# hall-lab/svtyper

Measured on AMD Instinct MI355X. Metric: breakpoints genotyped/sec, higher is better.
Workload: dtype f64

## Files before the change

### svtyper_amd/csrc/svt_batch_create.h

```cpp

struct StageTimer {
    bool on = std::getenv("SVT_TRACE") != nullptr;
    std::chrono::steady_clock::time_point t0 = std::chrono::steady_clock::now();
    void mark(const char* what)
    {
        if (!on) return;
        const auto t1 = std::chrono::steady_clock::now();
        std::fprintf(stderr, "[svt] %-28s %8.2f ms\n", what, std::chrono::duration<double, std::milli>(t1 - t0).count());
        t0 = t1;
    }
};

int record_error(uint32_t err_bits)
{
    return fail(SVT_ERR_INVALID, record_error_text(err_bits));
}

int check_stream_errors(svt_batch* b)
{
    if (b->layout != kLayoutStream || !b->d_err) return SVT_OK;
    uint32_t bits = 0;
    HIP_TRY(hipMemcpyAsync(&bits, b->d_err, sizeof(uint32_t), hipMemcpyDeviceToHost, b->stream));
    HIP_TRY(hipStreamSynchronize(b->stream));
    return bits ? record_error(bits) : SVT_OK;
// ... 310 lines not shown
    tables = (tables + 127) & ~size_t(127);
    if (single) {
        int wgs = 3;
        hipFuncAttributes fa{};
        if (hipFuncGetAttributes(&fa, stream_kernel_of(b, 1)) == hipSuccess && fa.numRegs > 0) wgs = std::max(1, std::min(8, 512 / ((fa.numRegs + 7) / 8 * 8)));
        else (void)hipGetLastError();
        const size_t by_lds = (160 * 1024) / (tables + kWavesPerBlock * kStreamRingBytes);
        b->one_tile_round_units = (uint64_t)std::min<size_t>((size_t)wgs, std::max<size_t>(by_lds, 1)) * cu_count(b->device) * kBlock;
    }
    {
        int wgs = 3;
        hipFuncAttributes fa{};
        if (hipFuncGetAttributes(&fa, b->mode == kMultiLds ? window_budget_kernel() : stream_kernel_of(b, tiles_per_wave(b, n))) == hipSuccess && fa.numRegs > 0)
            wgs = std::max(1, std::min(8, 512 / ((fa.numRegs + 7) / 8 * 8)));
        else
            (void)hipGetLastError();
        if (const char* e = std::getenv("SVT_STREAM_WGS_PER_CU")) wgs = std::max(1, std::atoi(e));
#ifdef SVT_FORCE_WGS
        wgs = SVT_FORCE_WGS;
#endif
        kStreamLdsPerWg = (160 * 1024 / (size_t)wgs) & ~size_t(127);
        b->wgs_per_cu = wgs;
    }
    const size_t l10_bytes = ((size_t)n_l10 * 8 + 127) & ~size_t(127);
    const size_t base_lds = tables + kWavesPerBlock * kStreamRingBytes;
    const size_t fit = std::max<size_t>(1, std::min<size_t>((size_t)b->wgs_per_cu, (160 * 1024) / base_lds));
    const size_t budget = ((160 * 1024) / fit) & ~size_t(127);
    (void)kStreamLdsPerWg;
    if (base_lds + l10_bytes <= budget) {
        a.l10_where = kL10Shared;
        a.lds_l10 = (uint32_t)tables;
        a.l10_lds_entries = n_l10;
        tables += l10_bytes;
    } else if (kStreamDepth == 1 && SVT_L10_THROUGH_RING) {
        a.l10_where = kL10Ring;
        a.l10_lds_entries = (uint32_t)std::min<uint64_t>((n_l10 + 127u) / 128u * 128u, kStreamRingBytes / 8);
    } else {
        a.l10_where = kL10Global;
        a.l10_lds_entries = 0;
    }
    a.lds_rings = (uint32_t)tables;
    if (b->mode == kSingleLds && a.l10_where != kL10Ring) {
        const size_t tab = (a.lds_winlibs + 127) & ~size_t(127);
        b->coop = small_region(tab, kCoopRegionBytes, true, l10_bytes, n_l10);
        if (b->coop.lds_bytes) {
            int wgs = 2;
            hipFuncAttributes fa{};
            if (hipFuncGetAttributes(&fa, coop_kernel_of(b)) == hipSuccess && fa.numRegs > 0) wgs = std::max(1, std::min(4, 512 / ((fa.numRegs + 7) / 8 * 8) * 4 / kCoopWaves));
            else (void)hipGetLastError();
            b->coop_resident = (uint32_t)std::min<size_t>((size_t)wgs, (160 * 1024) / b->coop.lds_bytes) * cu_count(b->device);
            if (b->coop.lds_bytes > 64 * 1024) HIP_TRY(hipFuncSetAttribute(coop_kernel_of(b), hipFuncAttributeMaxDynamicSharedMemorySize, (int)b->coop.lds_bytes));
        }
        b->split = small_region(tab, kSplitRegionBytes, true, l10_bytes, n_l10);
        if (b->split.lds_bytes > 64 * 1024)
            for (int lanes = 2; lanes <= 4; lanes += 2)
                HIP_TRY(hipFuncSetAttribute(split_kernel_of(b, lanes), hipFuncAttributeMaxDynamicSharedMemorySize, (int)b->split.lds_bytes));
    }
    if (b->mode == kMultiLds && a.l10_where != kL10Ring) {
        b->split = small_region((tables + 127) & ~size_t(127), kSplitRegionBytes, false);
        if (b->split.lds_bytes) {
            b->split.l10_where = a.l10_where;
            b->split.lds_l10 = a.lds_l10;
            b->split.l10_entries = a.l10_lds_entries;
        }
        if (b->split.lds_bytes > 64 * 1024)
            for (int lanes = 2; lanes <= 4; lanes += 2)
                if (lanes == 4 || !(b->flags & SVT_FLAG_SSO_ASSOCIATION))
                    HIP_TRY(hipFuncSetAttribute(split_kernel_of(b, lanes), hipFuncAttributeMaxDynamicSharedMemorySize, (int)b->split.lds_bytes));
    }
    a.n_units = n;
    a.unit_begin = 0;
    a.unit_end = (uint32_t)n;
    a.units_per_wg = (uint32_t)kBlock * (uint32_t)tiles_per_wave(b, n);
    a.result96 = (b->flags & SVT_FLAG_RESULT96) ? 1u : 0u;
    a.slot_begin = 0;
    b->resident_wgs = (uint32_t)std::min<size_t>((size_t)b->wgs_per_cu, (160 * 1024) / (tables + kWavesPerBlock * kStreamRingBytes)) *
                      cu_count(b->device);
    b->out_dev = b->d_out;
    b->out_slots = !a.result96 ? n : b->mode == kMultiLds ? (uint64_t)b->n_chunks * kBlock * (uint64_t)b->window_tiles : slots_of_launch(b, n);
    SVT_TRY(ensure_result_slots(b, b->out_slots));
    a.out = b->d_out;
    a.err = b->d_err;
    a.lib0 = T.libs[0];
    fill_gt_consts(a.c, in->split_weight, in->disc_weight);
    b->out_dev = b->d_out;
    b->lds_bytes = tables + kWavesPerBlock * kStreamRingBytes;
    if (b->lds_bytes > 160 * 1024) return fail(SVT_ERR_INVALID, "LDS budget exceeded");
    if (tm.on)
        std::fprintf(stderr, "[svt] kernel budget: %d workgroups/CU by registers, LDS %zu B/workgroup (%zu fit), log10 table (%u entries) %s (%u entries)\n",
                     b->wgs_per_cu, b->lds_bytes, (size_t)(160 * 1024) / std::max<size_t>(b->lds_bytes, 1), n_l10,
                     a.l10_where == kL10Shared ? "in LDS" : a.l10_where == kL10Ring ? "through the ring" : "through L2", a.l10_lds_entries);
    if (b->lds_bytes > 64 * 1024)
        for (int tiles = 1; tiles <= 2; ++tiles)
            if (b->mode != kGeneral || tiles == 1)
                HIP_TRY(hipFuncSetAttribute(stream_kernel_of(b, tiles), hipFuncAttributeMaxDynamicSharedMemorySize, (int)b->lds_bytes));
    if (b->lds_bytes > 64 * 1024 && b->split_window_kinds)
        for (int kind = 1; kind <= 2; ++kind)
            HIP_TRY(hipFuncSetAttribute(window_kernel_of_kind(kind), hipFuncAttributeMaxDynamicSharedMemorySize, (int)b->lds_bytes));
    return SVT_OK;
}
```

### svtyper_amd/csrc/svt_device_types.h

```cpp
#ifndef SVT_DEVICE_TYPES_H
#define SVT_DEVICE_TYPES_H

#include "svt_common.h"

namespace svt {

struct LibDesc {
    uint32_t tab_off;
    int32_t key_min;
    uint32_t n_bins;
    uint32_t pad;
    double v_nondel;
    double sd2;
};

constexpr uint32_t kHalfwordsPerRow = 8u;

constexpr uint32_t kErrStraddleNoPair = 2u, kErrLibIndex = 4u, kErrReservedBits = 8u, kErrNegativeSpan = 16u;

enum Layout : int {
    kLayoutStream = 3,
    kLayoutPacked = 4
};
struct Bin {
    int32_t thr;
    uint32_t hist;
};

constexpr uint32_t kLdsPm = 0;
constexpr uint32_t kLdsWtab = kLdsPm + 256 * 8;
constexpr uint32_t kLdsWcol = kLdsWtab + 32 * 16;
constexpr uint32_t kLdsWcolC = kLdsWcol + 2 * 32 * 8;
constexpr uint32_t kWcolRef = 32 * 8;
constexpr uint32_t kLdsBins = kLdsWcolC + 2 * 32 * 8;

struct GtConsts {
    double lgp[2][3];
    double lg1p[2][3];
    double ln10;
    double x_uflow;
    double split_weight;
    double disc_weight;
};

struct PairWeights { double w_alt, w_ref; };

enum LibMode : int {
    kSingleLds = 0,
    kMultiLds = 1,
    kGeneral = 2
};

struct WgDesc {
    uint32_t lib_lo, lib_cnt, bin_lo, bin_cnt;
};


}

#endif
```

### svtyper_amd/csrc/svt_host_tables.h

```cpp
#ifndef SVT_HOST_TABLES_H
#define SVT_HOST_TABLES_H

#include "svt_device_types.h"

namespace svt {


inline bool p_concordant_expr(uint32_t h1, uint32_t h2, uint64_t n_total)
{
    const double disc_prior = 0.05;
    const double conc_prior = 1 - disc_prior;
    const double d1 = h1 ? (double)h1 / (double)n_total : 0.0;
    const double d2 = h2 ? (double)h2 / (double)n_total : 0.0;
    const double den = conc_prior * d1 + disc_prior * d2;
    if (den == 0.0) return false;
    const double p = d1 * conc_prior / den;
    return p > 0.5;
}

inline double py_log10(double x) { return std::log(x) / std::log(10.0); }

inline double find_pow10_underflow()
{
    double lo = -330.0, hi = -300.0;
    for (int it = 0; it < 200; ++it) {
        double mid = lo + (hi - lo) / 2;
        if (mid == lo || mid == hi) break;
        if (std::pow(10.0, mid) > 0.0) hi = mid; else lo = mid;
    }
    while (std::pow(10.0, std::nextafter(hi, -INFINITY)) > 0.0) hi = std::nextafter(hi, -INFINITY);
    return hi;
}

inline void fill_gt_consts(GtConsts& c, double split_weight, double disc_weight)
{
    const double p_alt[2][3] = {{1e-3, 0.5, 0.9}, {1e-2, 0.2, 1 / 3.0}};
    for (int d = 0; d < 2; ++d)
        for (int g = 0; g < 3; ++g) {
            c.lgp[d][g] = py_log10(p_alt[d][g]);
            c.lg1p[d][g] = py_log10(1 - p_alt[d][g]);
        }
    c.ln10 = std::log(10.0);
    c.x_uflow = find_pow10_underflow();
    c.split_weight = split_weight;
    c.disc_weight = disc_weight;
}


struct HostTables {
    std::vector<LibDesc> libs;
    std::vector<Bin> bins;
    std::vector<PairWeights> wtab;
    std::vector<double> pm;
    std::vector<double> l10;
    bool fast_geometry = true;
    bool narrow_bins = true;
};

inline int build_tables(const svt_evidence_batch* in, uint64_t max_records_per_unit, HostTables& T)
{
    T.libs.resize(in->n_libs);
    for (uint32_t l = 0; l < in->n_libs; ++l) {
        const svt_library& L = in->libs[l];
        if (!L.hist || L.n_bins == 0) return fail(SVT_ERR_INVALID, "library without histogram");
        if (L.n_bins > (1u << 24)) return fail(SVT_ERR_INVALID, "histogram too wide");
        if (!std::isfinite(L.mean) || !std::isfinite(L.sd)) return fail(SVT_ERR_INVALID, "library moments not finite");
        uint64_t total = 0;
        uint32_t hmax = 0;
        for (uint32_t i = 0; i < L.n_bins; ++i) {
            if (L.hist[i] > 0x7FFFFFFFu) return fail(SVT_ERR_INVALID, "histogram count too large");
            total += L.hist[i];
            hmax = std::max(hmax, L.hist[i]);
        }
        LibDesc d{};
        d.tab_off = (uint32_t)T.bins.size();
        d.key_min = L.key_min;
        d.n_bins = L.n_bins;
        d.v_nondel = L.mean + L.sd * 3;
        d.sd2 = 2 * L.sd;
        T.libs[l] = d;
        if (L.key_min < -(1 << 29) || L.key_min > (1 << 29)) T.fast_geometry = false;
        if (!(std::fabs(d.v_nondel - std::nearbyint(d.v_nondel)) > 4e-6) || !(std::fabs(d.v_nondel) < 1e12))
            T.fast_geometry = false;
        for (uint32_t i = 0; i < L.n_bins; ++i) {
            const uint32_t h1 = L.hist[i];
            int32_t t = -1;
            if (h1 > 0 && total > 0 && p_concordant_expr(h1, 0, total)) {
                uint32_t lo = 0, hi = hmax;
                if (p_concordant_expr(h1, hi, total)) lo = hi;
                else
                    while (hi - lo > 1) {
                        const uint32_t mid = lo + (hi - lo) / 2;
                        if (p_concordant_expr(h1, mid, total)) lo = mid; else hi = mid;
                    }
                t = (int32_t)lo;
            }
            T.bins.push_back(Bin{t, h1});
        }
        T.bins.push_back(Bin{-1, 0u});
        {
            Bin* lb = T.bins.data() + d.tab_off;
            std::vector<uint32_t> vals;
            vals.reserve(2 * (size_t)L.n_bins + 2);
            for (uint32_t i = 0; i <= L.n_bins; ++i) {
                vals.push_back(lb[i].hist);
                if (lb[i].thr >= 0) vals.push_back((uint32_t)lb[i].thr);
            }
            std::sort(vals.begin(), vals.end());
            vals.erase(std::unique(vals.begin(), vals.end()), vals.end());
            auto rank = [&](const uint32_t x) { return (uint32_t)(std::lower_bound(vals.begin(), vals.end(), x) - vals.begin()); };
            for (uint32_t i = 0; i <= L.n_bins; ++i) {
                lb[i].hist = rank(lb[i].hist);
                if (lb[i].thr >= 0) lb[i].thr = (int32_t)rank((uint32_t)lb[i].thr);
            }
            if (vals.size() > 32767) T.narrow_bins = false;
        }
    }
    T.wtab.resize(32);
    for (int i = 0; i < 32; ++i) {
        const bool alt = i & 1, ra = i & 2, rb = i & 4, pc = i & 8, del = i & 16;
        const bool both = ra && rb, any = ra || rb;
        const bool need = any && (!both || del);
        T.wtab[i].w_alt = (alt && !(del && pc)) ? 1.0 : 0.0;
        T.wtab[i].w_ref = (need && pc) ? (both ? 1.0 : 0.5) : 0.0;
    }
    const double bound = 2.0 * (2.0 * in->split_weight + in->disc_weight) * (double)max_records_per_unit + 4.0;
    if (bound > 64.0 * 1024 * 1024) return fail(SVT_ERR_INVALID, "weights * records too large for the log table");
    T.l10.resize((size_t)bound + 1);
    T.l10[0] = 0.0;
    for (size_t i = 1; i < T.l10.size(); ++i) T.l10[i] = py_log10((double)i);
    T.pm.resize(256);
    for (int q = 0; q < 256; ++q) T.pm[q] = 1.0 - std::pow(10.0, -(double)q / 10.0);
    return SVT_OK;
}


}

#endif
```

### svtyper_amd/csrc/svt_stream_kernel.h

```cpp
#ifndef SVT_STREAM_KERNEL_H
#define SVT_STREAM_KERNEL_H

#ifndef SVT_STREAM_AUX
#define SVT_STREAM_AUX 2
#endif
#ifndef SVT_STREAM_EDGE_AUX
#define SVT_STREAM_EDGE_AUX 0
#endif
#ifndef SVT_STREAM_SPLIT
#define SVT_STREAM_SPLIT 4
#endif
#ifndef SVT_STREAM_WAVES
#define SVT_STREAM_WAVES 3
#endif
#ifndef SVT_WINDOW_WAVES
#define SVT_WINDOW_WAVES 3
#endif

#include <type_traits>

#include "svt_wg_parts.h"

namespace svt {

template <int MODE>
struct RecordCheck {
    uint32_t flags_or = 0, span_or = 0, lone = 0, lib_max = 0;
    __device__ __forceinline__ void see(const u32x4 w, const uint32_t lib_key = 0u)
    {
        if (MODE == kMultiLds) flags_or |= w.w ^ lib_key;
        else flags_or |= w.w;
        span_or |= w.x;
        lone = max(lone, (w.w & 0x17u) ^ 0x10u);
        if (MODE == kGeneral) lib_max = max(lib_max, w.w & 0xffff00u);
    }
    __device__ __forceinline__ void window_lib(const uint32_t d) { lib_max = max(lib_max, d); }
    __device__ __forceinline__ uint32_t bits(const uint32_t limit) const
    {
        const uint32_t n_libs = limit;
        const bool bad_lib = MODE == kSingleLds ? (flags_or & 0xffff00u) != 0u
                             : MODE == kMultiLds ? (limit == 1u ? (flags_or & 0xffff00u) != 0u : lib_max >= limit)
                                                 : (lib_max >> SVT_REC_LIB_SHIFT) >= n_libs;
        return (lone > 0x10u ? kErrStraddleNoPair : 0u) | (bad_lib ? kErrLibIndex : 0u) |
               ((flags_or & ~SVT_REC_FLAG_MASK) ? kErrReservedBits : 0u) | ((int32_t)span_or < 0 ? kErrNegativeSpan : 0u);
    }
};

template <bool SSO, bool EDGE, bool CONT = true>
__device__ __forceinline__ double record_weights(const u32x4 w, const bool mine, Acc& a)
{
    const uint32_t wy = EDGE ? (mine ? w.y : 0u) : w.y;
    const uint32_t wz = EDGE ? (mine ? w.z : 0u) : w.z;
    const double pm_a = lds_f64(kSPm + byte0_x8(wy)), pm_b = lds_f64(kSPm + byte1_x8(wy));
    const double rs_a = lds_f64(kSPm + byte2_x8(wy)), rs_b = lds_f64(kSPm + byte3_x8(wy));
    const double p_seq = lds_f64(kSPmHalf + byte0_x8(wz)) + lds_f64(kSPmHalf + byte1_x8(wz));
    const double p_clip = lds_f64(kSPmHalf + byte2_x8(wz)) + lds_f64(kSPmHalf + byte3_x8(wz));
    if (SSO && !CONT) {
        a.ref_seq += a.l_ref_seq;
        a.alt_seq += a.l_alt_seq;
        a.alt_clip += a.l_alt_clip;
        a.l_ref_seq = rs_a + rs_b;
        a.l_alt_seq = p_seq;
        a.l_alt_clip = p_clip;
    } else if (SSO) {
        const bool cont = (w.w & SVT_REC_CONTINUATION) != 0u;
        a.ref_seq += cont ? 0.0 : a.l_ref_seq;
        a.alt_seq += cont ? 0.0 : a.l_alt_seq;
        a.alt_clip += cont ? 0.0 : a.l_alt_clip;
        a.l_ref_seq = ((cont ? a.l_ref_seq : 0.0) + rs_a) + rs_b;
        a.l_alt_seq = (cont ? a.l_alt_seq : 0.0) + p_seq;
        a.l_alt_clip = (cont ? a.l_alt_clip : 0.0) + p_clip;
    } else {
        a.ref_seq = (a.ref_seq + rs_a) + rs_b;
        a.alt_seq += p_seq;
        a.alt_clip += p_clip;
    }
    return pm_a * pm_b;
}

template <bool SSO, bool EDGE, bool CONT>
__device__ __forceinline__ void record_single(const u32x4 w, const bool mine, const StreamCtx& c, Acc& a)
{
    const double pp = record_weights<SSO, EDGE, CONT>(w, mine, a);
    const uint32_t i1 = min(w.x - c.kmin, c.nb), i2 = min(w.x - c.sub2, c.nb);
    const int32_t thr1 = lds_i16(kSBins + (i1 << 1));
    const uint32_t h2 = lds_u16(c.hist_at + (i2 << 1));
    const bool p_conc = (int32_t)h2 <= thr1;
    const uint32_t wa = (p_conc ? c.wt1 : c.wt0) | ((w.w & c.fmask) << 3);
    a.alt_span += pp * lds_f64(wa);
    a.ref_span += pp * lds_f64(wa + kSWref);
}

struct WindowCtx {
    uint32_t lib_lo;
    uint32_t lib_last;
    uint32_t winlibs_at;
    uint32_t vl_or_never;
    uint32_t wt0, wt1;
    uint32_t wh0;
    uint32_t gated;
    bool is_del;
};

typedef __attribute__((address_space(3))) const u32x4 lds_cu32x4;

template <bool SSO, bool EDGE, bool CONT, class CHECK>
__device__ __forceinline__ void record_window(const u32x4 w, const bool mine, const WindowCtx& c, Acc& a, CHECK& check)
{
    const double pp = record_weights<SSO, EDGE, CONT>(w, mine, a);
    check.window_lib(EDGE && !mine ? 0u : SVT_REC_LIB(w.w) - c.lib_lo);
    const uint32_t la = c.winlibs_at + min(SVT_REC_LIB(w.w) - c.lib_lo, c.lib_last) * (uint32_t)sizeof(WinLib);
    const u32x4 d = *reinterpret_cast<lds_cu32x4*>((size_t)la);
    const uint32_t open = (uint32_t)__builtin_amdgcn_sbfe((int32_t)c.gated, min(SVT_REC_LIB(w.w) - c.lib_lo, c.lib_last), 1u);
    const uint32_t f3 = w.w & 7u & open;
    const uint32_t sub2 = c.vl_or_never + d.x;
    const uint32_t i1 = min(w.x - d.x, d.y), i2 = min(w.x - sub2, d.y);
    const int32_t thr1 = lds_i16(d.z + (i1 << 1));
    const uint32_t h2 = lds_u16(d.w + (i2 << 1));
    const bool p_conc = (int32_t)h2 <= thr1;
    const uint32_t wa = (p_conc ? c.wt1 : c.wt0) | (f3 << 3);
    a.alt_span += pp * lds_f64(wa);
    a.ref_span += pp * lds_f64(wa + kSWref);
}

template <bool SSO, int MODE, int R, int WK = 0>
__global__ __launch_bounds__(kBlock, MODE == kSingleLds ? SVT_STREAM_WAVES : MODE == kMultiLds ? (WK ? 4 : SVT_WINDOW_WAVES) : 2) void svt_stream_kernel(const StreamArgs a)
{
    static_assert(WK == 0 || (MODE == kMultiLds && !SSO), "window kinds: classic library-window kernels only");
    extern __shared__ __attribute__((aligned(16))) unsigned char smem[];
    constexpr uint32_t kUnitsPerWg = kBlock * R;
    if (MODE != kGeneral && (uint32_t)(size_t)(__attribute__((address_space(3))) unsigned char*)smem != 0u) __builtin_trap();
    unsigned char* rings = smem + a.lds_rings;
    const uint32_t tid = threadIdx.x, lane = tid % kWave;
    const uint32_t wave = (uint32_t)__builtin_amdgcn_readfirstlane((int)(tid / kWave));
    const WgUnits g = wg_units<MODE>(a);
    const uint32_t wg_base = g.wg_base, n_here = g.n_here, wg_index = g.wg_index;
    const WgDesc wd = g.wd;
    auto unit_at = [&](const uint32_t local) -> uint32_t { return wg_unit_at<MODE>(a, wg_base, local); };

    uint32_t beg[R], cnt[R];
#pragma unroll
    for (int j = 0; j < R; ++j) {
        const uint32_t local = (uint32_t)j * kBlock + tid;
        beg[j] = 0u;
        cnt[j] = 0u;
        if (local < n_here) {
            const uint32_t u = unit_at(local);
            const uint64_t lo = a.rec_offset[u], hi = a.rec_offset[u + 1];
            beg[j] = (uint32_t)lo;
            cnt[j] = (uint32_t)(hi - lo);
        }
    }

    stage_tables<MODE, kBlock, true>(smem, a, wd, tid);
    uint4 info[R];
    wg_sort_into_tiles<R>(rings, beg, cnt, n_here, tid, lane, wave, info);

    Tables t;
    t.pm = reinterpret_cast<double*>(smem + kSPm);
    t.wtab = reinterpret_cast<PairWeights*>(smem + kSWtab);
    t.libs = reinterpret_cast<LibDesc*>(smem + kSBins);
    t.bins = a.bins;

    unsigned char* ring = rings + wave * kStreamRingBytes;
    const uint32_t ring_addr = (uint32_t)(size_t)(__attribute__((address_space(3))) unsigned char*)ring;
    const uint32_t o = lane >> 3, rr = lane & 7u;
    const uint32_t col_even = (rr ^ (o >> 1)) << 4, col_odd = col_even ^ 64u;
    const uint32_t sw = (lane >> 1) & 7u;
    const uint32_t lane_block = ring_addr + lane * 128u, sw16 = sw << 4;
    const char* rec_bytes = reinterpret_cast<const char*>(a.records);

    RecordCheck<MODE> check;
    const uint32_t lib_key = MODE == kMultiLds && wd.lib_cnt == 1u ? wd.lib_lo << SVT_REC_LIB_SHIFT : 0u;

#pragma unroll
    for (int r = 0; r < R; ++r) {
        const uint32_t first_rec = info[r].x, n_rec = info[r].y;
        const uint32_t unit = info[r].z == kPadUnit ? kPadUnit : unit_at(info[r].z);
        svt_unit U{};
        if (unit != kPadUnit) U = a.units[unit];
        const uint32_t head = first_rec & 7u, last = head + n_rec;
        const uint32_t nblk = n_rec ? (last + 7u) >> 3 : 0u;
        uint32_t max_blk, min_blk;
        tile_block_range(nblk, max_blk, min_blk);
        uint32_t src_first[8], src_end[8], src_base[8];
#pragma unroll
        for (int i = 0; i < 8; ++i) {
            src_first[i] = (uint32_t)__shfl((int)first_rec, 8 * i + (int)o, kWave);
            src_end[i] = src_first[i] + (uint32_t)__shfl((int)n_rec, 8 * i + (int)o, kWave);
            src_base[i] = (src_first[i] & ~7u) + (((i & 1) ? col_odd : col_even) >> 4);
        }

        constexpr int kEdgeAux = R >= 2 ? SVT_STREAM_EDGE_AUX : SVT_STREAM_AUX;
        auto fetch_first = [&]() {
            fetch_block<kEdgeAux, true>(0, src_base, src_first, src_end, rec_bytes, ring);
        };
        auto fetch = [&](const uint32_t k, const uint32_t st = 0u) -> bool {
            unsigned char* stage = ring + st * kStageBytes;
            if (k + 1 < min_blk) {
                fetch_block_interior<SVT_STREAM_AUX>(k, src_base, rec_bytes, stage);
                return true;
            } else if (kEdgeAux != SVT_STREAM_AUX && k + 1 >= min_blk) {
                constexpr bool kLastUseInLastTile = R >= 2;
                if (kLastUseInLastTile && r == R - 1) fetch_block_tail_exact<SVT_STREAM_AUX, SVT_STREAM_AUX>(k, src_base, src_end, rec_bytes, stage);
                else fetch_block_tail_exact<SVT_STREAM_AUX, kEdgeAux>(k, src_base, src_end, rec_bytes, stage);
            } else
                fetch_block<SVT_STREAM_AUX, false>(k, src_base, src_first, src_end, rec_bytes, stage);
            return false;
        };

        LaneCtx c{};
        c.is_del = U.svtype == SVT_SVTYPE_DEL;
        c.del16 = c.is_del ? 16u : 0u;
        c.var_length = U.var_length;
        c.pos_delta_d = (double)U.pos_delta;
        StreamCtx sc;
        {
            const bool small_del = c.is_del && (c.pos_delta_d < a.lib0.sd2);
            sc.fmask = small_del ? 0u : 7u;
            sc.kmin = (uint32_t)a.lib0.key_min;
            sc.nb = a.lib0.n_bins;
            sc.sub2 = c.is_del ? (uint32_t)U.var_length + (uint32_t)a.lib0.key_min : 0x80000000u;
            sc.hist_at = kSBins + a.total_bins * 2u;
            sc.wt0 = kSWtab + c.del16 * 8u;
            sc.wt1 = sc.wt0 + 8u * 8u;
            sc.wh0 = kSWhi + c.del16 * 4u;
        }
        if (MODE == kMultiLds) {
            const WinLib w0 = reinterpret_cast<const WinLib*>(smem + a.lds_winlibs)[0];
            const bool small_del = c.is_del && (c.pos_delta_d < w0.sd2);
            sc.fmask = small_del ? 0u : 7u;
            sc.kmin = w0.kmin;
            sc.nb = w0.nb;
            sc.sub2 = c.is_del ? (uint32_t)U.var_length + w0.kmin : 0x80000000u;
            sc.hist_at = w0.hist_at;
        }
        WindowCtx wc;
        wc.lib_lo = wd.lib_lo;
        wc.lib_last = wd.lib_cnt - 1u;
        wc.winlibs_at = a.lds_winlibs;
        wc.vl_or_never = c.is_del ? (uint32_t)U.var_length : 0x80000000u;
        wc.wt0 = sc.wt0;
        wc.wt1 = sc.wt1;
        wc.wh0 = sc.wh0;
        wc.is_del = c.is_del;
        wc.gated = 0u;
        if (MODE == kMultiLds && c.is_del) {
            for (uint32_t l = 0; l < wd.lib_cnt; ++l)
                wc.gated |= (c.pos_delta_d < reinterpret_cast<const WinLib*>(smem + a.lds_winlibs)[l].sd2 ? 1u : 0u) << l;
        }
        wc.gated = ~wc.gated;
        Acc acc = {0.0, 0.0, 0.0, 0.0, 0.0, 0.0, 0.0, 0.0};

        auto consume = [&](const u32x4 (&w)[8], const uint32_t k, auto edge, auto window_kind, auto continuations) {
            constexpr bool EDGE = decltype(edge)::value;
            constexpr bool CONT = decltype(continuations)::value;
            constexpr int KIND = decltype(window_kind)::value;
            auto is_mine = [&](const int j) -> bool {
                const uint32_t idx = k * kBlockRecords + (uint32_t)j;
                return !EDGE || (idx >= head && idx < last);
            };
#pragma unroll
            for (int j = 0; j < 8; ++j) {
                if (j == SVT_STREAM_SPLIT) __builtin_amdgcn_sched_barrier(0);
                const bool mine = is_mine(j);
                const u32x4 wj = w[j];
                if (mine) check.see(wj, lib_key);
                if (MODE == kSingleLds) {
                    record_single<SSO, EDGE, CONT>(wj, mine, sc, acc);
                } else if (MODE == kMultiLds) {
                    if (KIND == 1) record_single<SSO, EDGE, CONT>(wj, mine, sc, acc);
                    else record_window<SSO, EDGE, CONT>(wj, mine, wc, acc, check);
                } else {
                    const uint32_t wy = mine ? wj.y : 0u, wz = mine ? wj.z : 0u;
                    weight_evidence<SSO>(wy >> 16 | (wz << 16), wz >> 16, (wj.w & SVT_REC_CONTINUATION) != 0, t, acc);
                    pair_evidence(wj.x, wy & 0xffffu, wj.w & 7u, min(SVT_REC_LIB(wj.w), a.n_libs - 1u), t, c, acc);
                }
            }
        };

        auto l10_into_ring = [&]() {
            const char* l10_bytes = reinterpret_cast<const char*>(a.l10);
            for (uint32_t off = 0; off < a.l10_lds_entries * 8u; off += 1024u)
                __builtin_amdgcn_global_load_lds(l10_bytes + off + lane * 16u, (lds_void_ptr)(ring + off), 16, 0, 0);
        };
        if (max_blk) {
            fetch_first();
            u32x4 w[8];
            bool exact_behind = false;
            if (kStreamDepth == 2 && max_blk > 1) exact_behind = fetch(1, 1);
#pragma unroll 1
            for (uint32_t k = 0; k < max_blk; ++k) {
                const uint32_t stage_off = kStreamDepth == 2 ? (k & 1u) * kStageBytes : 0u;
                if (kStreamDepth == 2) {
                    const bool pend = k + 1 < max_blk && exact_behind;
                    if (k & 1u) {
                        if (pend) read_block<kStageBytes, 8>(lane_block, sw16, w);
                        else read_block<kStageBytes, 0>(lane_block, sw16, w);
                    } else {
                        if (pend) read_block<0, 8>(lane_block, sw16, w);
                        else read_block<0, 0>(lane_block, sw16, w);
                    }
                } else {
                    read_block(lane_block, sw16, w);
                }
                auto refill = [&]() {
                    if (kStreamDepth == 2) {
                        if (k + 2 < max_blk) exact_behind = fetch(k + 2, k & 1u);
                    } else if (k + 1 < max_blk) fetch(k + 1);
                    else if (a.l10_where == kL10Ring) l10_into_ring();
                };
                const uint32_t k8 = k * kBlockRecords;
                const uint32_t neutral_w = MODE == kMultiLds ? wd.lib_lo << SVT_REC_LIB_SHIFT : 0u;
                if (__any(k8 < head || k8 + kBlockRecords > last)) {
#pragma unroll
                    for (int j = 0; j < 8; ++j) {
                        const bool mine = k8 + (uint32_t)j - head < n_rec;
                        w[j].x = mine ? w[j].x : 0u;
                        w[j].y = mine ? w[j].y : 0u;
                        w[j].z = mine ? w[j].z : 0u;
                        w[j].w = mine ? w[j].w : neutral_w;
                    }
                }
                bool has_cont = false;
                if (SSO && MODE != kGeneral)
                    has_cont = __any(((w[0].w | w[1].w | w[2].w | w[3].w | w[4].w | w[5].w | w[6].w | w[7].w) & SVT_REC_CONTINUATION) != 0u);
                if (SSO && MODE != kGeneral && has_cont) {
#pragma unroll 1
                    for (uint32_t j = 0; j < 8u; ++j) {
                        u32x4 wj = *reinterpret_cast<lds_cu32x4*>((size_t)(lane_block + stage_off + ((j << 4) ^ sw16)));
                        const bool mine = k8 + j - head < n_rec;
                        wj.x = mine ? wj.x : 0u;
                        wj.y = mine ? wj.y : 0u;
                        wj.z = mine ? wj.z : 0u;
                        wj.w = mine ? wj.w : neutral_w;
                        check.see(wj, lib_key);
                        if (MODE == kSingleLds || WK == 1 || (WK == 0 && !SSO && wd.lib_cnt == 1u)) record_single<SSO, false, true>(wj, true, sc, acc);
                        else record_window<SSO, false, true>(wj, true, wc, acc, check);
                    }
                    refill();
                    continue;
                }
                refill();
                using kind_any = std::integral_constant<int, 0>;
                using kind_one = std::integral_constant<int, 1>;
                auto run = [&](auto edge_tag, auto kind_tag) {
                    if (!SSO || MODE == kGeneral || has_cont) consume(w, k, edge_tag, kind_tag, std::true_type{});
                    else consume(w, k, edge_tag, kind_tag, std::false_type{});
                };
                if (MODE == kMultiLds && WK != 2 && (WK == 1 || (!SSO && wd.lib_cnt == 1u))) run(std::false_type{}, kind_one{});
                else run(std::false_type{}, kind_any{});
            }
        }
        if (SSO) {
            acc.ref_seq += acc.l_ref_seq;
            acc.alt_seq += acc.l_alt_seq;
            acc.alt_clip += acc.l_alt_clip;
        }

        const double* lds_l10 = reinterpret_cast<const double*>(a.l10_where == kL10Shared ? smem + a.lds_l10 : ring);
        if (a.l10_where == kL10Ring) {
            if (!max_blk || kStreamDepth == 2) l10_into_ring();
            asm volatile("s_waitcnt vmcnt(0)" ::: "memory");
        }
        uint4 piece[8];
        unit_epilogue(acc, (uint32_t)U.svtype, (uint32_t)U.flags, a.c, lds_l10, a.l10, a.l10_lds_entries, piece);

        uint32_t unit_out = unit;
        if (a.out_samples > 1u && unit != kPadUnit) {
            const uint32_t sample = unit / a.out_sites;
            unit_out = (unit - sample * a.out_sites) * a.out_samples + sample;
        }
        uint32_t tile_slot = 0xFFFFFFFFu;
        if (a.result96) {
            result96_tag(piece, unit_out);
            tile_slot = a.slot_begin + wg_index * kUnitsPerWg + ((uint32_t)r * kWavesPerBlock + ((r & 1) ? (uint32_t)kWavesPerBlock - 1u - wave : wave)) * kWave;
        }
        store_result_records_through_ring(ring, piece, unit_out, lane, reinterpret_cast<unsigned char*>(a.out), a.result96 ? 6u : 8u, tile_slot);
    }
    const uint32_t bad = check.bits(MODE == kMultiLds ? wd.lib_cnt : a.n_libs);
    if (bad) atomicOr(a.err, bad);
}

}

#endif
```

### svtyper_amd/csrc/svt_unit_math.h

```cpp
#ifndef SVT_UNIT_MATH_H
#define SVT_UNIT_MATH_H

#include "svt_device_types.h"
#include "svt_entry_formats.h"

namespace svt {

typedef __attribute__((address_space(3))) const double lds_cf64;
typedef __attribute__((address_space(3))) const uint32_t lds_cu32;
typedef __attribute__((address_space(3))) const int32_t lds_ci32;

__device__ __forceinline__ double lds_f64(const uint32_t addr) { return *reinterpret_cast<lds_cf64*>((size_t)addr); }
__device__ __forceinline__ uint32_t lds_u32(const uint32_t addr) { return *reinterpret_cast<lds_cu32*>((size_t)addr); }
__device__ __forceinline__ int32_t lds_i32(const uint32_t addr) { return *reinterpret_cast<lds_ci32*>((size_t)addr); }
typedef __attribute__((address_space(3))) const int16_t lds_ci16;
typedef __attribute__((address_space(3))) const uint16_t lds_cu16;
__device__ __forceinline__ int32_t lds_i16(const uint32_t addr) { return *reinterpret_cast<lds_ci16*>((size_t)addr); }
__device__ __forceinline__ uint32_t lds_u16(const uint32_t addr) { return *reinterpret_cast<lds_cu16*>((size_t)addr); }

#define SVT_BYTE_X8(N)                                                                                       \
    __device__ __forceinline__ uint32_t byte##N##_x8(const uint32_t e)                                      \
    {                                                                                                        \
        uint32_t r;                                                                                          \
        asm("v_lshlrev_b32_sdwa %0, %1, %2 dst_sel:DWORD dst_unused:UNUSED_PAD src0_sel:DWORD src1_sel:BYTE_" #N \
            : "=v"(r) : "v"(3u), "v"(e));                                                                    \
        return r;                                                                                            \
    }
SVT_BYTE_X8(0)
SVT_BYTE_X8(1)
SVT_BYTE_X8(2)
SVT_BYTE_X8(3)
#undef SVT_BYTE_X8

struct Tables {
    const double* pm;
    const PairWeights* wtab;
    const LibDesc* libs;
    const Bin* bins;
};

struct Acc {
    double ref_seq, alt_seq, alt_clip, ref_span, alt_span;
    double l_ref_seq, l_alt_seq, l_alt_clip;
};

struct LaneCtx {
    uint32_t del16;
    int32_t var_length;
    double pos_delta_d;
    bool is_del;
    uint32_t wt0, wt1;
    uint32_t common_mq;
    uint32_t nb4, off2_4;
    uint32_t hist_at;
    uint32_t tab8;
    uint32_t libs_at;
    uint32_t lib_last;
};

template <bool SSO>
__device__ __forceinline__ void weight_evidence(const uint32_t wa, const uint32_t wb, const bool cont,
                                                const Tables& t, Acc& a)
{
    const double rs_a = t.pm[wa & 0xffu];
    const double rs_b = t.pm[(wa >> 8) & 0xffu];
    const double sq_l = t.pm[(wa >> 16) & 0xffu];
    const double sq_r = t.pm[wa >> 24];
    const double cl_l = t.pm[wb & 0xffu];
    const double cl_r = t.pm[(wb >> 8) & 0xffu];
    const double p_seq = (sq_l + sq_r) * 0.5;
    const double p_clip = (cl_l + cl_r) * 0.5;
    if (SSO) {
        a.ref_seq += cont ? 0.0 : a.l_ref_seq;
        a.alt_seq += cont ? 0.0 : a.l_alt_seq;
        a.alt_clip += cont ? 0.0 : a.l_alt_clip;
        a.l_ref_seq = ((cont ? a.l_ref_seq : 0.0) + rs_a) + rs_b;
        a.l_alt_seq = (cont ? a.l_alt_seq : 0.0) + p_seq;
        a.l_alt_clip = (cont ? a.l_alt_clip : 0.0) + p_clip;
    } else {
        a.ref_seq = (a.ref_seq + rs_a) + rs_b;
        a.alt_seq += p_seq;
        a.alt_clip += p_clip;
    }
}

__device__ __forceinline__ void pair_evidence(const uint32_t o, const uint32_t mq, uint32_t f3,
                                              const uint32_t lib_idx, const Tables& t, const LaneCtx& c, Acc& a)
{
    const double pm_a = t.pm[mq & 0xffu];
    const double pm_b = t.pm[(mq >> 8) & 0xffu];

    int32_t thr1;
    uint32_t h2;
    {
        const LibDesc lib = t.libs[lib_idx];
        const bool small_del = c.is_del && (c.pos_delta_d < lib.sd2);
        f3 = small_del ? 0u : f3;
        const int64_t i1 = (int64_t)(int32_t)o - (int64_t)lib.key_min;
        const bool in1 = (uint64_t)i1 < (uint64_t)lib.n_bins;
        thr1 = t.bins[lib.tab_off + (in1 ? (uint32_t)i1 : lib.n_bins)].thr;
        int64_t key2;
        bool ok2 = true;
        if (c.is_del) {
            key2 = (int64_t)(int32_t)o - (int64_t)c.var_length;
        } else {
            const double kf = (double)(int32_t)o - lib.v_nondel;
            ok2 = (kf == floor(kf)) && (fabs(kf) < 4.0e9);
            key2 = ok2 ? (int64_t)kf : 0;
        }
        const int64_t i2 = key2 - (int64_t)lib.key_min;
        const bool in2 = ok2 && ((uint64_t)i2 < (uint64_t)lib.n_bins);
        h2 = t.bins[lib.tab_off + (in2 ? (uint32_t)i2 : lib.n_bins)].hist;
    }
    const bool p_conc = (int32_t)h2 <= thr1;
    const PairWeights pw = t.wtab[f3 | (p_conc ? 8u : 0u) | c.del16];
    const double pp = pm_a * pm_b;
    a.alt_span += pp * pw.w_alt;
    a.ref_span += pp * pw.w_ref;
}

template <int MULTI>
__device__ __forceinline__ void pair_tables(const uint32_t code4, const LaneCtx& c, const Bin* bins, int32_t& thr1, uint32_t& h2)
{
    if (MULTI) {
        const char* base = reinterpret_cast<const char*>(bins) + c.tab8;
        thr1 = *reinterpret_cast<const int32_t*>(base + 2u * min(code4, c.nb4));
        h2 = *reinterpret_cast<const uint32_t*>(base + 2u * min(code4 - c.off2_4, c.nb4) + 4u);
    } else {
        thr1 = lds_i32(kLdsBins + min(code4, c.nb4));
        h2 = lds_u32(c.hist_at + min(code4 - c.off2_4, c.nb4));
    }
}

constexpr int kOneLibrary = 0, kLibsInLds = 1, kLibsInHbm = 2;

template <int MULTI>
__device__ __forceinline__ void enter_library(const uint32_t l, LaneCtx& c, const LibDesc* libs)
{
    uint32_t tab_off, n_bins;
    if (MULTI == kLibsInHbm) {
        const uint4 d = *reinterpret_cast<const uint4*>(libs + min(l, c.lib_last));
        tab_off = d.x;
        n_bins = d.z;
    } else {
        const uint32_t at = c.libs_at + min(l, c.lib_last) * (uint32_t)sizeof(LibDesc);
        tab_off = lds_u32(at);
        n_bins = lds_u32(at + 8u);
    }
    c.tab8 = tab_off * (uint32_t)sizeof(Bin);
    c.nb4 = n_bins * 4u;
    c.off2_4 = c.is_del ? min((uint32_t)c.var_length, n_bins) * 4u : 0x80000000u;
}

template <int MULTI>
__device__ __forceinline__ void switch_library(const uint32_t h, LaneCtx& c, const LibDesc* libs)
{
    if ((h & 0x8007u) == 0u && h != 0u) enter_library<MULTI>((h >> 3) - 1u, c, libs);
}

template <int MULTI>
__device__ __forceinline__ void pair_eval_single(const uint32_t code4, const uint32_t f3x8, const double pp,
                                                 const LaneCtx& c, Acc& a, const Bin* bins)
{
    int32_t thr1;
    uint32_t h2;
    pair_tables<MULTI>(code4, c, bins, thr1, h2);
    const bool p_conc = (int32_t)h2 <= thr1;
    const uint32_t wa = (p_conc ? c.wt1 : c.wt0) | f3x8;
    const double w_alt = lds_f64(wa), w_ref = lds_f64(wa + kWcolRef);
    a.alt_span += pp * w_alt;
    a.ref_span += pp * w_ref;
}

template <int MULTI>
__device__ __forceinline__ void short_pair_dword(const uint32_t e, LaneCtx& c, Acc& a, const Bin* bins, const LibDesc* libs)
{
    const bool wide = (e & 0x8000u) != 0u;
    const uint32_t hi = e >> 16;
    const uint32_t mq = wide ? hi : c.common_mq;
    const double pm_a = lds_f64(kLdsPm + byte0_x8(mq)), pm_b = lds_f64(kLdsPm + byte1_x8(mq));
    if (MULTI) switch_library<MULTI>(e & 0xffffu, c, libs);
    if (MULTI == kLibsInHbm && (e & 0xffffu) == kWideSwitch) enter_library<MULTI>(hi, c, libs);
    pair_eval_single<MULTI>((e >> 1) & 0x3ffcu, (e << 3) & 0x38u, pm_a * pm_b, c, a, bins);
    if (MULTI && !wide) switch_library<MULTI>(hi, c, libs);
    {
        const uint32_t code4 = (e >> 17) & 0x3ffcu;
        int32_t thr1;
        uint32_t h2;
        pair_tables<MULTI>(code4, c, bins, thr1, h2);
        const bool p_conc = (int32_t)h2 <= thr1;
        const uint32_t wa = ((p_conc ? c.wt1 : c.wt0) + (kLdsWcolC - kLdsWcol)) | (wide ? 0u : (e >> 13) & 0x38u);
        a.alt_span += lds_f64(wa);
        a.ref_span += lds_f64(wa + kWcolRef);
    }
}

template <bool SSO>
__device__ __forceinline__ void ref_read_pair(const double x, const double y, const bool first, Acc& a)
{
    if (SSO) {
        a.ref_seq += first ? a.l_ref_seq : 0.0;
// ... 181 lines not shown
```

### svtyper_amd/csrc/svt_wg_parts.h

```cpp
#ifndef SVT_WG_PARTS_H
#define SVT_WG_PARTS_H

#include "svt_ring_engine.h"

namespace svt {

constexpr uint32_t kSPm = 0;
constexpr uint32_t kSPmHalf = kSPm + 256 * 8;
constexpr uint32_t kSWtab = kSPmHalf + 256 * 8;
constexpr uint32_t kSWref = 32 * 8;
constexpr uint32_t kSWhi = kSWtab + 2 * 32 * 8;
constexpr uint32_t kSWhiRef = 32 * 4;
constexpr uint32_t kSBins = kSWhi + 2 * 32 * 4;

struct StreamArgs {
    const uint4* records;
    const uint64_t* rec_offset;
    const svt_unit* units;
    const double* pm;
    const double* l10;
    const LibDesc* libs;
    const Bin* bins;
    const PairWeights* wtab;
    uint32_t n_l10;
    uint32_t n_libs;
    uint32_t total_bins;
    uint32_t last_blk;
    uint32_t lds_bins;
    uint32_t lds_libs;
    uint32_t lds_rings;
    uint32_t l10_where;
    uint32_t lds_l10;
    uint32_t l10_lds_entries;
    uint64_t n_units;
    svt_result* out;
    uint32_t* err;
    const uint32_t* perm;
    const uint2* chunks;
    const WgDesc* windows;
    uint32_t lds_winlibs;
    uint32_t unit_begin;
    uint32_t unit_end;
    uint32_t units_per_wg;
    uint32_t chunk_begin;
    uint32_t result96;
    uint32_t slot_begin;
    uint32_t out_samples;
    uint32_t out_sites;
    LibDesc lib0;
    GtConsts c;
};

struct WinLib {
    uint32_t kmin;
    uint32_t nb;
    uint32_t thr_at;
    uint32_t hist_at;
    double sd2;
    double pad;
};
static_assert(sizeof(WinLib) == 32, "WinLib is read as two 16-byte halves");

struct WgUnits {
    uint32_t wg_index;
    uint32_t wg_base;
    uint32_t n_here;
    WgDesc wd;
};
template <int MODE>
__device__ __forceinline__ WgUnits wg_units(const StreamArgs& a, const uint32_t chunk_cap = 0xFFFFFFFFu)
{
    WgUnits g;
    g.wg_base = a.unit_begin + blockIdx.x * a.units_per_wg;
    g.wd = WgDesc{};
    g.wg_index = MODE == kMultiLds ? blockIdx.x + a.chunk_begin : blockIdx.x;
    if (MODE == kMultiLds) {
        const uint2 ch = a.chunks[g.wg_index];
        g.wg_base = ch.x;
        g.n_here = min(ch.y, chunk_cap);
        g.wd = a.windows[g.wg_index];
    } else {
        g.n_here = min(a.units_per_wg, a.unit_end - g.wg_base);
    }
    return g;
}
template <int MODE>
__device__ __forceinline__ uint32_t wg_unit_at(const StreamArgs& a, const uint32_t wg_base, const uint32_t local)
{
    return MODE == kMultiLds && a.perm ? a.perm[wg_base + local] : wg_base + local;
}

template <int MODE, uint32_t THREADS, bool HI>
__device__ __forceinline__ void stage_tables(unsigned char* smem, const StreamArgs& a, const WgDesc& wd, const uint32_t tid)
{
    for (uint32_t i = tid; i < 256; i += THREADS) {
        const double p = a.pm[i];
        reinterpret_cast<double*>(smem + kSPm)[i] = p;
        reinterpret_cast<double*>(smem + kSPmHalf)[i] = p * 0.5;
    }
    if (tid < 32) {
        const PairWeights pw = a.wtab[tid];
        if (MODE != kGeneral) {
            reinterpret_cast<double*>(smem + kSWtab)[tid] = pw.w_alt;
            reinterpret_cast<double*>(smem + kSWtab + kSWref)[tid] = pw.w_ref;
            if (HI) {
                reinterpret_cast<uint32_t*>(smem + kSWhi)[tid] = (uint32_t)__double2hiint(pw.w_alt);
                reinterpret_cast<uint32_t*>(smem + kSWhi + kSWhiRef)[tid] = (uint32_t)__double2hiint(pw.w_ref);
            }
        } else {
            reinterpret_cast<PairWeights*>(smem + kSWtab)[tid] = pw;
        }
    }
    if (MODE == kSingleLds) {
        int16_t* s_thr = reinterpret_cast<int16_t*>(smem + kSBins);
        uint16_t* s_hst = reinterpret_cast<uint16_t*>(smem + kSBins) + a.total_bins;
        for (uint32_t i = tid; i < a.total_bins; i += THREADS) {
            const Bin bn = a.bins[i];
            s_thr[i] = (int16_t)bn.thr;
            s_hst[i] = (uint16_t)bn.hist;
        }
    } else if (MODE == kMultiLds) {
        int16_t* s_thr = reinterpret_cast<int16_t*>(smem + kSBins);
        uint16_t* s_hst = reinterpret_cast<uint16_t*>(smem + kSBins) + wd.bin_cnt;
        for (uint32_t i = tid; i < wd.bin_cnt; i += THREADS) {
            const Bin bn = a.bins[wd.bin_lo + i];
            s_thr[i] = (int16_t)bn.thr;
            s_hst[i] = (uint16_t)bn.hist;
        }
        if (tid < wd.lib_cnt) {
            const LibDesc L = a.libs[wd.lib_lo + tid];
            WinLib wl;
            wl.kmin = (uint32_t)L.key_min;
            wl.nb = L.n_bins;
            wl.thr_at = kSBins + (L.tab_off - wd.bin_lo) * 2u;
            wl.hist_at = kSBins + (wd.bin_cnt + L.tab_off - wd.bin_lo) * 2u;
            wl.sd2 = L.sd2;
            wl.pad = 0.0;
            reinterpret_cast<WinLib*>(smem + a.lds_winlibs)[tid] = wl;
        }
    } else {
        for (uint32_t i = tid; i < a.n_libs * (uint32_t)(sizeof(LibDesc) / 8); i += THREADS)
            reinterpret_cast<uint64_t*>(smem + kSBins)[i] = reinterpret_cast<const uint64_t*>(a.libs)[i];
    }
    if (a.l10_where == kL10Shared) {
        double* s_l10 = reinterpret_cast<double*>(smem + a.lds_l10);
        for (uint32_t i = tid; i < a.n_l10; i += THREADS) s_l10[i] = a.l10[i];
    }
}

struct StreamCtx {
    uint32_t fmask;
    uint32_t kmin;
    uint32_t nb;
    uint32_t sub2;
    uint32_t hist_at;
    uint32_t wt0, wt1;
    uint32_t wh0;
};

constexpr uint32_t kTileFmask = 7u, kTileDel16 = 16u, kTileSvtypeShift = 8u, kTileUflagsShift = 16u;
template <int MODE>
__device__ __forceinline__ uint4 make_tile_entry(const svt_unit& U, const uint32_t beg, const uint32_t cnt, const StreamArgs& a)
{
    const bool is_del = U.svtype == SVT_SVTYPE_DEL;
    const bool small_del = MODE == kSingleLds && is_del && ((double)U.pos_delta < a.lib0.sd2);
    const uint32_t flags = (small_del ? 0u : kTileFmask) | (is_del ? kTileDel16 : 0u) | ((uint32_t)U.svtype << kTileSvtypeShift) |
                           ((uint32_t)U.flags << kTileUflagsShift);
    const uint32_t sub2 = is_del ? (uint32_t)U.var_length + (MODE == kSingleLds ? (uint32_t)a.lib0.key_min : 0u) : 0x80000000u;
    return make_uint4(beg, cnt, sub2, flags);
}
__device__ __forceinline__ uint32_t tile_svtype(const uint32_t flags) { return (flags >> kTileSvtypeShift) & 0xffu; }
__device__ __forceinline__ uint32_t tile_uflags(const uint32_t flags) { return flags >> kTileUflagsShift; }

__device__ __forceinline__ uint32_t result_destination(const StreamArgs& a, const uint32_t unit)
{
    uint32_t unit_out = unit;
    if (a.out_samples > 1u && unit != kPadUnit) {
        const uint32_t sample = unit / a.out_sites;
        unit_out = (unit - sample * a.out_sites) * a.out_samples + sample;
    }
    return unit_out;
}
__device__ __forceinline__ void tally_epilogue(const StreamArgs& a, const unsigned char* smem, const double* s_tally, const uint4* s_tile,
                                               const uint32_t* s_unit, const uint32_t p, unsigned char* ring, const uint32_t lane,
                                               const uint32_t tile_slot)
{
    Acc acc = {s_tally[p], s_tally[kBlock + p], s_tally[2 * kBlock + p], s_tally[3 * kBlock + p], s_tally[4 * kBlock + p], 0.0, 0.0, 0.0};
    const uint32_t unit = s_unit[p], flags = s_tile[p].w;
    const double* lds_l10 = reinterpret_cast<const double*>(smem + a.lds_l10);
    uint4 piece[8];
    unit_epilogue(acc, tile_svtype(flags), tile_uflags(flags), a.c, lds_l10, a.l10, a.l10_where == kL10Shared ? a.l10_lds_entries : 0u, piece);
    const uint32_t unit_out = result_destination(a, unit);
    uint32_t sorted_base = 0xFFFFFFFFu;
// ... 11 lines not shown
```

Baseline: 3.448 billion.

## Add fast 32-bit general-mode record path with per-block exact fallback

Adds a per-library fast-geometry flag and a streamlined record_general path for the multi-library general kernel. It uses 32-bit clamped bin indexing, reads library descriptors straight from LDS and uses the split weight-column layout shared with the other modes. Blocks whose records touch non-fast libraries, carry huge variant lengths or hold continuation records fall back to a scalar exact path. The general kernel's occupancy bound becomes a macro defaulting to 3 waves. The cost is extra branch and flag checks per block, and correctness now relies on the 32-bit index clamping being equivalent for the flagged libraries.

```diff
diff --git a/svtyper_amd/csrc/svt_batch_create.h b/svtyper_amd/csrc/svt_batch_create.h
--- a/svtyper_amd/csrc/svt_batch_create.h
+++ b/svtyper_amd/csrc/svt_batch_create.h
@@ -416,6 +416,7 @@
     a.out = b->d_out;
     a.err = b->d_err;
     a.lib0 = T.libs[0];
+    a.exact_libs = T.exact_libs ? 1u : 0u;
     fill_gt_consts(a.c, in->split_weight, in->disc_weight);
     b->out_dev = b->d_out;
     b->lds_bytes = tables + kWavesPerBlock * kStreamRingBytes;
diff --git a/svtyper_amd/csrc/svt_device_types.h b/svtyper_amd/csrc/svt_device_types.h
--- a/svtyper_amd/csrc/svt_device_types.h
+++ b/svtyper_amd/csrc/svt_device_types.h
@@ -9,10 +9,12 @@
     uint32_t tab_off;
     int32_t key_min;
     uint32_t n_bins;
-    uint32_t pad;
+    uint32_t flags;
     double v_nondel;
     double sd2;
 };
+
+constexpr uint32_t kLibFast32 = 1u;
 
 constexpr uint32_t kHalfwordsPerRow = 8u;
 
diff --git a/svtyper_amd/csrc/svt_host_tables.h b/svtyper_amd/csrc/svt_host_tables.h
--- a/svtyper_amd/csrc/svt_host_tables.h
+++ b/svtyper_amd/csrc/svt_host_tables.h
@@ -55,6 +55,7 @@
     std::vector<double> l10;
     bool fast_geometry = true;
     bool narrow_bins = true;
+    bool exact_libs = false;
 };
 
 inline int build_tables(const svt_evidence_batch* in, uint64_t max_records_per_unit, HostTables& T)
@@ -79,9 +80,13 @@
         d.v_nondel = L.mean + L.sd * 3;
         d.sd2 = 2 * L.sd;
         T.libs[l] = d;
-        if (L.key_min < -(1 << 29) || L.key_min > (1 << 29)) T.fast_geometry = false;
+        bool fast = true;
+        if (L.key_min < -(1 << 29) || L.key_min > (1 << 29)) fast = false;
         if (!(std::fabs(d.v_nondel - std::nearbyint(d.v_nondel)) > 4e-6) || !(std::fabs(d.v_nondel) < 1e12))
-            T.fast_geometry = false;
+            fast = false;
+        if (!fast) T.fast_geometry = false;
+        if (fast && std::isfinite(d.sd2) && (uint64_t)d.tab_off + L.n_bins + 1 <= (1ull << 32) / sizeof(Bin)) T.libs[l].flags = kLibFast32;
+        else T.exact_libs = true;
         for (uint32_t i = 0; i < L.n_bins; ++i) {
             const uint32_t h1 = L.hist[i];
             int32_t t = -1;
diff --git a/svtyper_amd/csrc/svt_stream_kernel.h b/svtyper_amd/csrc/svt_stream_kernel.h
--- a/svtyper_amd/csrc/svt_stream_kernel.h
+++ b/svtyper_amd/csrc/svt_stream_kernel.h
@@ -15,6 +15,10 @@
 #endif
 #ifndef SVT_WINDOW_WAVES
 #define SVT_WINDOW_WAVES 3
+#endif
+
+#ifndef SVT_GENERAL_WAVES
+#define SVT_GENERAL_WAVES 3
 #endif
 
 #include <type_traits>
@@ -123,13 +127,45 @@
     a.ref_span += pp * lds_f64(wa + kSWref);
 }
 
+struct GeneralCtx {
+    uint32_t vl;
+    uint32_t never;
+    uint32_t wt0, wt1;
+    double gate_pd;
+};
+
+template <bool SSO, bool EDGE, bool CONT>
+__device__ __forceinline__ void record_general(const u32x4 w, const bool mine, const GeneralCtx& c, const uint32_t lib_last,
+                                               const char* bins, Acc& a)
+{
+    const double pp = record_weights<SSO, EDGE, CONT>(w, mine, a);
+    const uint32_t la = kSBins + min(SVT_REC_LIB(w.w), lib_last) * (uint32_t)sizeof(LibDesc);
+    const u32x4 d = *reinterpret_cast<lds_cu32x4*>((size_t)la);
+    const bool small_del = c.gate_pd < lds_f64(la + 24u);
+    const uint32_t f3 = small_del ? 0u : w.w & 7u;
+    const uint32_t i1 = min(w.x - d.y, d.z), i2 = min((w.x - (c.vl + d.y)) | c.never, d.z);
+    const int32_t thr1 = *reinterpret_cast<const int32_t*>(bins + (size_t)((d.x + i1) * (uint32_t)sizeof(Bin)));
+    const uint32_t h2 = *reinterpret_cast<const uint32_t*>(bins + (size_t)((d.x + i2) * (uint32_t)sizeof(Bin)) + 4);
+    const bool p_conc = (int32_t)h2 <= thr1;
+    const uint32_t wa = (p_conc ? c.wt1 : c.wt0) | (f3 << 3);
+    a.alt_span += pp * lds_f64(wa);
+    a.ref_span += pp * lds_f64(wa + kSWref);
+}
+
+template <bool SSO>
+__device__ __forceinline__ void record_exact(const u32x4 w, const LaneCtx& c, const uint32_t lib_last, const Bin* bins, Acc& a)
+{
+    const double pp = record_weights<SSO, false, true>(w, true, a);
+    pair_evidence(w.x, w.w & 7u, kSBins + min(SVT_REC_LIB(w.w), lib_last) * (uint32_t)sizeof(LibDesc), pp, bins, c, a);
+}
+
 template <bool SSO, int MODE, int R, int WK = 0>
-__global__ __launch_bounds__(kBlock, MODE == kSingleLds ? SVT_STREAM_WAVES : MODE == kMultiLds ? (WK ? 4 : SVT_WINDOW_WAVES) : 2) void svt_stream_kernel(const StreamArgs a)
+__global__ __launch_bounds__(kBlock, MODE == kSingleLds ? SVT_STREAM_WAVES : MODE == kMultiLds ? (WK ? 4 : SVT_WINDOW_WAVES) : SVT_GENERAL_WAVES) void svt_stream_kernel(const StreamArgs a)
 {
     static_assert(WK == 0 || (MODE == kMultiLds && !SSO), "window kinds: classic library-window kernels only");
     extern __shared__ __attribute__((aligned(16))) unsigned char smem[];
     constexpr uint32_t kUnitsPerWg = kBlock * R;
-    if (MODE != kGeneral && (uint32_t)(size_t)(__attribute__((address_space(3))) unsigned char*)smem != 0u) __builtin_trap();
+    if ((uint32_t)(size_t)(__attribute__((address_space(3))) unsigned char*)smem != 0u) __builtin_trap();
     unsigned char* rings = smem + a.lds_rings;
     const uint32_t tid = threadIdx.x, lane = tid % kWave;
     const uint32_t wave = (uint32_t)__builtin_amdgcn_readfirstlane((int)(tid / kWave));
@@ -155,12 +191,6 @@
     stage_tables<MODE, kBlock, true>(smem, a, wd, tid);
     uint4 info[R];
     wg_sort_into_tiles<R>(rings, beg, cnt, n_here, tid, lane, wave, info);
-
-    Tables t;
-    t.pm = reinterpret_cast<double*>(smem + kSPm);
-    t.wtab = reinterpret_cast<PairWeights*>(smem + kSWtab);
-    t.libs = reinterpret_cast<LibDesc*>(smem + kSBins);
-    t.bins = a.bins;
 
     unsigned char* ring = rings + wave * kStreamRingBytes;
     const uint32_t ring_addr = (uint32_t)(size_t)(__attribute__((address_space(3))) unsigned char*)ring;
@@ -214,6 +244,16 @@
         c.del16 = c.is_del ? 16u : 0u;
         c.var_length = U.var_length;
         c.pos_delta_d = (double)U.pos_delta;
+        c.wt0 = kSWtab + c.del16 * 8u;
+        c.wt1 = c.wt0 + 8u * 8u;
+        GeneralCtx gc;
+        gc.vl = (uint32_t)U.var_length;
+        gc.never = c.is_del ? 0u : 0xFFFFFFFFu;
+        gc.wt0 = c.wt0;
+        gc.wt1 = c.wt1;
+        gc.gate_pd = c.is_del ? c.pos_delta_d : __builtin_huge_val();
+        const bool exact_unit = c.is_del && (U.var_length < -(1 << 30) || U.var_length > (1 << 30));
+        const uint32_t lib_last = a.n_libs - 1u;
         StreamCtx sc;
         {
             const bool small_del = c.is_del && (c.pos_delta_d < a.lib0.sd2);
@@ -272,9 +312,7 @@
                     if (KIND == 1) record_single<SSO, EDGE, CONT>(wj, mine, sc, acc);
                     else record_window<SSO, EDGE, CONT>(wj, mine, wc, acc, check);
                 } else {
-                    const uint32_t wy = mine ? wj.y : 0u, wz = mine ? wj.z : 0u;
-                    weight_evidence<SSO>(wy >> 16 | (wz << 16), wz >> 16, (wj.w & SVT_REC_CONTINUATION) != 0, t, acc);
-                    pair_evidence(wj.x, wy & 0xffffu, wj.w & 7u, min(SVT_REC_LIB(wj.w), a.n_libs - 1u), t, c, acc);
+                    record_general<SSO, EDGE, CONT>(wj, mine, gc, lib_last, reinterpret_cast<const char*>(a.bins), acc);
                 }
             }
         };
@@ -323,8 +361,34 @@
                     }
                 }
                 bool has_cont = false;
-                if (SSO && MODE != kGeneral)
+                if (SSO)
                     has_cont = __any(((w[0].w | w[1].w | w[2].w | w[3].w | w[4].w | w[5].w | w[6].w | w[7].w) & SVT_REC_CONTINUATION) != 0u);
+                bool exact_blk = false;
+                if (MODE == kGeneral) {
+                    bool lane_exact = exact_unit;
+                    if (a.exact_libs) {
+                        uint32_t fast = kLibFast32;
+#pragma unroll
+                        for (int j = 0; j < 8; ++j) fast &= lds_u32(kSBins + min(SVT_REC_LIB(w[j].w), lib_last) * (uint32_t)sizeof(LibDesc) + 12u);
+                        lane_exact = lane_exact || !fast;
+                    }
+                    exact_blk = __any(lane_exact) || has_cont;
+                }
+                if (MODE == kGeneral && exact_blk) {
+#pragma unroll 1
+                    for (uint32_t j = 0; j < 8u; ++j) {
+                        u32x4 wj = *reinterpret_cast<lds_cu32x4*>((size_t)(lane_block + stage_off + ((j << 4) ^ sw16)));
+                        const bool mine = k8 + j - head < n_rec;
+                        wj.x = mine ? wj.x : 0u;
+                        wj.y = mine ? wj.y : 0u;
+                        wj.z = mine ? wj.z : 0u;
+                        wj.w = mine ? wj.w : 0u;
+                        check.see(wj);
+                        record_exact<SSO>(wj, c, lib_last, a.bins, acc);
+                    }
+                    refill();
+                    continue;
+                }
                 if (SSO && MODE != kGeneral && has_cont) {
 #pragma unroll 1
                     for (uint32_t j = 0; j < 8u; ++j) {
@@ -345,7 +409,7 @@
                 using kind_any = std::integral_constant<int, 0>;
                 using kind_one = std::integral_constant<int, 1>;
                 auto run = [&](auto edge_tag, auto kind_tag) {
-                    if (!SSO || MODE == kGeneral || has_cont) consume(w, k, edge_tag, kind_tag, std::true_type{});
+                    if (!SSO || has_cont) consume(w, k, edge_tag, kind_tag, std::true_type{});
                     else consume(w, k, edge_tag, kind_tag, std::false_type{});
                 };
                 if (MODE == kMultiLds && WK != 2 && (WK == 1 || (!SSO && wd.lib_cnt == 1u))) run(std::false_type{}, kind_one{});
diff --git a/svtyper_amd/csrc/svt_unit_math.h b/svtyper_amd/csrc/svt_unit_math.h
--- a/svtyper_amd/csrc/svt_unit_math.h
+++ b/svtyper_amd/csrc/svt_unit_math.h
@@ -31,13 +31,6 @@
 SVT_BYTE_X8(2)
 SVT_BYTE_X8(3)
 #undef SVT_BYTE_X8
-
-struct Tables {
-    const double* pm;
-    const PairWeights* wtab;
-    const LibDesc* libs;
-    const Bin* bins;
-};
 
 struct Acc {
     double ref_seq, alt_seq, alt_clip, ref_span, alt_span;
@@ -58,47 +51,23 @@
     uint32_t lib_last;
 };
 
-template <bool SSO>
-__device__ __forceinline__ void weight_evidence(const uint32_t wa, const uint32_t wb, const bool cont,
-                                                const Tables& t, Acc& a)
-{
-    const double rs_a = t.pm[wa & 0xffu];
-    const double rs_b = t.pm[(wa >> 8) & 0xffu];
-    const double sq_l = t.pm[(wa >> 16) & 0xffu];
-    const double sq_r = t.pm[wa >> 24];
-    const double cl_l = t.pm[wb & 0xffu];
-    const double cl_r = t.pm[(wb >> 8) & 0xffu];
-    const double p_seq = (sq_l + sq_r) * 0.5;
-    const double p_clip = (cl_l + cl_r) * 0.5;
-    if (SSO) {
-        a.ref_seq += cont ? 0.0 : a.l_ref_seq;
-        a.alt_seq += cont ? 0.0 : a.l_alt_seq;
-        a.alt_clip += cont ? 0.0 : a.l_alt_clip;
-        a.l_ref_seq = ((cont ? a.l_ref_seq : 0.0) + rs_a) + rs_b;
-        a.l_alt_seq = (cont ? a.l_alt_seq : 0.0) + p_seq;
-        a.l_alt_clip = (cont ? a.l_alt_clip : 0.0) + p_clip;
-    } else {
-        a.ref_seq = (a.ref_seq + rs_a) + rs_b;
-        a.alt_seq += p_seq;
-        a.alt_clip += p_clip;
-    }
-}
-
-__device__ __forceinline__ void pair_evidence(const uint32_t o, const uint32_t mq, uint32_t f3,
-                                              const uint32_t lib_idx, const Tables& t, const LaneCtx& c, Acc& a)
-{
-    const double pm_a = t.pm[mq & 0xffu];
-    const double pm_b = t.pm[(mq >> 8) & 0xffu];
-
+__device__ __forceinline__ void pair_evidence(const uint32_t o, uint32_t f3, const uint32_t lib_at, const double pp,
+                                              const Bin* bins, const LaneCtx& c, Acc& a)
+{
     int32_t thr1;
     uint32_t h2;
     {
-        const LibDesc lib = t.libs[lib_idx];
+        LibDesc lib;
+        lib.tab_off = lds_u32(lib_at);
+        lib.key_min = lds_i32(lib_at + 4u);
+        lib.n_bins = lds_u32(lib_at + 8u);
+        lib.v_nondel = lds_f64(lib_at + 16u);
+        lib.sd2 = lds_f64(lib_at + 24u);
         const bool small_del = c.is_del && (c.pos_delta_d < lib.sd2);
         f3 = small_del ? 0u : f3;
         const int64_t i1 = (int64_t)(int32_t)o - (int64_t)lib.key_min;
         const bool in1 = (uint64_t)i1 < (uint64_t)lib.n_bins;
-        thr1 = t.bins[lib.tab_off + (in1 ? (uint32_t)i1 : lib.n_bins)].thr;
+        thr1 = bins[lib.tab_off + (in1 ? (uint32_t)i1 : lib.n_bins)].thr;
         int64_t key2;
         bool ok2 = true;
         if (c.is_del) {
@@ -110,13 +79,12 @@
         }
         const int64_t i2 = key2 - (int64_t)lib.key_min;
         const bool in2 = ok2 && ((uint64_t)i2 < (uint64_t)lib.n_bins);
-        h2 = t.bins[lib.tab_off + (in2 ? (uint32_t)i2 : lib.n_bins)].hist;
+        h2 = bins[lib.tab_off + (in2 ? (uint32_t)i2 : lib.n_bins)].hist;
     }
     const bool p_conc = (int32_t)h2 <= thr1;
-    const PairWeights pw = t.wtab[f3 | (p_conc ? 8u : 0u) | c.del16];
-    const double pp = pm_a * pm_b;
-    a.alt_span += pp * pw.w_alt;
-    a.ref_span += pp * pw.w_ref;
+    const uint32_t wa = (p_conc ? c.wt1 : c.wt0) | (f3 << 3);
+    a.alt_span += pp * lds_f64(wa);
+    a.ref_span += pp * lds_f64(wa + kWcolRef);
 }
 
 template <int MULTI>
diff --git a/svtyper_amd/csrc/svt_wg_parts.h b/svtyper_amd/csrc/svt_wg_parts.h
--- a/svtyper_amd/csrc/svt_wg_parts.h
+++ b/svtyper_amd/csrc/svt_wg_parts.h
@@ -49,6 +49,7 @@
     uint32_t out_sites;
     LibDesc lib0;
     GtConsts c;
+    uint32_t exact_libs;
 };
 
 struct WinLib {
@@ -100,15 +101,11 @@
     }
     if (tid < 32) {
         const PairWeights pw = a.wtab[tid];
-        if (MODE != kGeneral) {
-            reinterpret_cast<double*>(smem + kSWtab)[tid] = pw.w_alt;
-            reinterpret_cast<double*>(smem + kSWtab + kSWref)[tid] = pw.w_ref;
-            if (HI) {
-                reinterpret_cast<uint32_t*>(smem + kSWhi)[tid] = (uint32_t)__double2hiint(pw.w_alt);
-                reinterpret_cast<uint32_t*>(smem + kSWhi + kSWhiRef)[tid] = (uint32_t)__double2hiint(pw.w_ref);
-            }
-        } else {
-            reinterpret_cast<PairWeights*>(smem + kSWtab)[tid] = pw;
+        reinterpret_cast<double*>(smem + kSWtab)[tid] = pw.w_alt;
+        reinterpret_cast<double*>(smem + kSWtab + kSWref)[tid] = pw.w_ref;
+        if (HI && MODE != kGeneral) {
+            reinterpret_cast<uint32_t*>(smem + kSWhi)[tid] = (uint32_t)__double2hiint(pw.w_alt);
+            reinterpret_cast<uint32_t*>(smem + kSWhi + kSWhiRef)[tid] = (uint32_t)__double2hiint(pw.w_ref);
         }
     }
     if (MODE == kSingleLds) {
```

Result: slower. 3.387 billion (-1.8%).
